# TheShadow29/VidSitu

Hardware: AMD Instinct MI355X
Metric: clips/s (10s@32x224x224) SlowFast+TxEnc fwd+bwd (higher is better)
Workload: dtype bf16

## Files before the change

### vidsitu_amd/csrc/conv_wgrad.hip

```cpp
#include <stdlib.h>

#include "common.h"

#include <mutex>
#include <type_traits>
#include "glue_bodies.h"

typedef __attribute__((ext_vector_type(4))) short s16x4;
typedef __attribute__((address_space(3))) s16x4 lds_s16x4;

struct WgradP {
  const uint16_t* dy;
  const uint16_t* x;
  float* out;
  int P;
  int Cout, Kp, Cin, x_ld, dy_ld;
  int To, Ho, Wo, Ti, Hi, Wi;
  int kT, kH, kW, sT, sH, sW, pT, pH, pW;
  int tilesM, tilesN, S, rows_per_split;
  unsigned x_bytes, dy_bytes;
  int xcd_order;
  int dbg;
};

#define WG_OOB 0x80000000u

#define WG_ROWTAB 1024

__device__ __forceinline__ int wg_swz_chunk(int row) {
  return ((row & 3) << 1) | (((row >> 3) & 1) << 3);
}

#ifndef WG_NARROW_DEPTH
#define WG_NARROW_DEPTH 3
#endif
constexpr int wg_depth(int bm) { return bm <= 32 ? WG_NARROW_DEPTH : 2; }

template <int BM, int BN, int WM, int WN, int MODE>
__global__ __launch_bounds__(256) void conv_wgrad_kernel(WgradP p) {
  extern __shared__ __attribute__((aligned(16))) char smem[];
  constexpr int D = wg_depth(BM), R = D - 1;
  static_assert(D >= 2 && R * 64 < WG_ROWTAB / 2, "loads never run past the table half being rebuilt");
  constexpr int TM = BM / WM, TN = BN / WN;
  constexpr int MR = TM / 16, NR = TN / 16;
  constexpr int CM = BM / 8, CN = BN / 8;
  constexpr int RPM = 256 / CM, RPN = 256 / CN;
  constexpr int IM = (64 + RPM - 1) / RPM, IN = (64 + RPN - 1) / RPN;
  constexpr int IMG = 64 * 256;
  constexpr int STAGE = 2 * IMG;
  static_assert(WM * WN == 4, "4 waves");

  const int tid = threadIdx.x;
  int bid = blockIdx.x;
  if (p.xcd_order) {
    const int nwg = gridDim.x, q = nwg >> 3, r = nwg & 7, xcd = blockIdx.x & 7;
    bid = (xcd < r ? xcd * (q + 1) : r * (q + 1) + (xcd - r) * q) + (blockIdx.x >> 3);
  }
  const int ntile = p.tilesM * p.tilesN;
  const int s = bid / ntile;
  bid -= s * ntile;
  const int tn = bid % p.tilesN, tm = bid / p.tilesN;
  const int m0 = tm * BM, n0 = tn * BN;
  const int pbeg = s * p.rows_per_split;
  const int pend = min(p.P, pbeg + p.rows_per_split);

  int4* rowtab = (int4*)(smem + 2 * STAGE);

  const int ccm = tid % CM, rm = tid / CM;
  const int ccn = tid % CN, rn = tid / CN;
  const bool mcol_ok = (m0 + ccm * 8) < p.Cout;
  const int ncol = n0 + ccn * 8;
  const bool ncol_ok = ncol < p.Kp;
  int dt = 0, dh = 0, dw = 0, c0 = 0;
  if (MODE == 1 && ncol_ok) {
    const int tap = ncol / p.Cin;
    c0 = ncol - tap * p.Cin;
    dw = tap % p.kW;
    const int t2 = tap / p.kW;
    dh = t2 % p.kH;
    dt = t2 / p.kH;
  }

  u32x4 ra[R][IM], rb[R][IN];
  const __amdgpu_buffer_rsrc_t xsrc =
      __builtin_amdgcn_make_buffer_rsrc((void*)p.x, 0, (int)p.x_bytes, 0x00020000);
  const __amdgpu_buffer_rsrc_t dysrc =
      __builtin_amdgcn_make_buffer_rsrc((void*)p.dy, 0, (int)p.dy_bytes, 0x00020000);
  const unsigned dycol = (unsigned)((m0 + ccm * 8) * 2);
  const unsigned xtap = (MODE == 1)
      ? (unsigned)(((((long long)dt * p.Hi + dh) * p.Wi + dw) * p.x_ld + c0) * 2)
      : (unsigned)(ncol * 2);

  auto gload_a = [&](int u, int pstep) __attribute__((always_inline)) {
#pragma unroll
    for (int i = 0; i < IM; ++i) {
      const int r = rm + RPM * i;
      const int pp = pstep + r;
      const unsigned ok = (unsigned)(r < 64) & (unsigned)mcol_ok & (unsigned)(pp < pend);
      const unsigned off = ok ? (unsigned)pp * (unsigned)(p.dy_ld * 2) + dycol : WG_OOB;
      ra[u][i] = __builtin_bit_cast(u32x4, __builtin_amdgcn_raw_buffer_load_b128(dysrc, off, 0, 0));
    }
  };
  auto gload_b = [&](int u, int pstep) __attribute__((always_inline)) {
#pragma unroll
    for (int i = 0; i < IN; ++i) {
      const int r = rn + RPN * i;
      const int pp = pstep + r;
      unsigned ok = (unsigned)(r < 64) & (unsigned)ncol_ok & (unsigned)(pp < pend);
      unsigned off;
      if (MODE == 0) {
        off = (unsigned)pp * (unsigned)(p.x_ld * 2) + xtap;
      } else {
        const int4 e = rowtab[(pp - pbeg) & (WG_ROWTAB - 1)];
        const int ti = e.y + dt, hi = e.z + dh, wi = e.w + dw;
        ok &= (unsigned)((unsigned)ti < (unsigned)p.Ti) & (unsigned)((unsigned)hi < (unsigned)p.Hi) &
              (unsigned)((unsigned)wi < (unsigned)p.Wi);
        off = (unsigned)e.x + xtap;
      }
      rb[u][i] = __builtin_bit_cast(u32x4, __builtin_amdgcn_raw_buffer_load_b128(xsrc, ok ? off : WG_OOB, 0, 0));
    }
  };

  auto sstore = [&](int u, int buf) __attribute__((always_inline)) {
    char* A = smem + buf * STAGE;
    char* B = A + IMG;
#pragma unroll
    for (int i = 0; i < IM; ++i) {
      const int r = rm + RPM * i;
      if (r < 64) *(u32x4*)(A + r * 256 + ((ccm ^ wg_swz_chunk(r)) << 4)) = ra[u][i];
    }
#pragma unroll
    for (int i = 0; i < IN; ++i) {
      const int r = rn + RPN * i;
      if (r < 64) *(u32x4*)(B + r * 256 + ((ccn ^ wg_swz_chunk(r)) << 4)) = rb[u][i];
    }
  };

  auto build_tab = [&](int rel0, int count) __attribute__((always_inline)) {
    for (int i = tid; i < count; i += 256) {
      const int pp = pbeg + rel0 + i;
      int4 e = make_int4(0, -(1 << 20), -(1 << 20), -(1 << 20));
      if (pp < pend) {
        int wo, t1, ho, t2, to, n;
        if (p.P < (1 << 24)) {
          fast_divmod(pp, p.Wo, 1.0f / (float)p.Wo, t1, wo);
          fast_divmod(t1, p.Ho, 1.0f / (float)p.Ho, t2, ho);
          fast_divmod(t2, p.To, 1.0f / (float)p.To, n, to);
        } else {
          wo = pp % p.Wo; t1 = pp / p.Wo;
          ho = t1 % p.Ho; t2 = t1 / p.Ho;
          to = t2 % p.To; n = t2 / p.To;
        }
        e.y = to * p.sT - p.pT;
        e.z = ho * p.sH - p.pH;
        e.w = wo * p.sW - p.pW;
        const long long pos0 = (((long long)n * p.Ti + e.y) * p.Hi + e.z) * p.Wi + e.w;
        e.x = (int)(unsigned)(pos0 * p.x_ld * 2);
      }
      rowtab[(rel0 + i) & (WG_ROWTAB - 1)] = e;
    }
  };

  const int wave = tid >> 6, lane = tid & 63;
  const int wm = wave / WN, wn = wave % WN;
  const int g = lane >> 4, li = lane & 15, q = li >> 2, pp4 = li & 3;

  f32x4 acc[MR][NR];
#pragma unroll
  for (int a = 0; a < MR; ++a)
#pragma unroll
    for (int b = 0; b < NR; ++b) acc[a][b] = (f32x4){0.f, 0.f, 0.f, 0.f};

  auto compute = [&](int buf) __attribute__((always_inline)) {
    const char* A = smem + buf * STAGE;
    const char* B = A + IMG;
#pragma unroll
    for (int ks = 0; ks < 2; ++ks) {
      const int row = ks * 32 + 8 * g + q;
      const int swz = ((row & 3) << 2) | (((row >> 3) & 1) << 4);
      bf16x8 af[MR], bfr[NR];
#pragma unroll
      for (int a = 0; a < MR; ++a) {
        const int unit = ((wm * TM + a * 16) >> 2) + pp4;
        const lds_s16x4* ptr = (const lds_s16x4*)(A + row * 256 + ((unit ^ swz) << 3));
        const s16x4 lo = __builtin_amdgcn_ds_read_tr16_b64_v4i16((lds_s16x4*)ptr);
        const s16x4 hi = __builtin_amdgcn_ds_read_tr16_b64_v4i16((lds_s16x4*)(ptr + 128));
        typedef __attribute__((ext_vector_type(8))) short s16x8;
        const s16x8 v = __builtin_shufflevector(lo, hi, 0, 1, 2, 3, 4, 5, 6, 7);
        af[a] = __builtin_bit_cast(bf16x8, v);
      }
#pragma unroll
      for (int b = 0; b < NR; ++b) {
        const int unit = ((wn * TN + b * 16) >> 2) + pp4;
        const lds_s16x4* ptr = (const lds_s16x4*)(B + row * 256 + ((unit ^ swz) << 3));
        const s16x4 lo = __builtin_amdgcn_ds_read_tr16_b64_v4i16((lds_s16x4*)ptr);
        const s16x4 hi = __builtin_amdgcn_ds_read_tr16_b64_v4i16((lds_s16x4*)(ptr + 128));
        typedef __attribute__((ext_vector_type(8))) short s16x8;
        const s16x8 v = __builtin_shufflevector(lo, hi, 0, 1, 2, 3, 4, 5, 6, 7);
        bfr[b] = __builtin_bit_cast(bf16x8, v);
      }
#pragma unroll
      for (int a = 0; a < MR; ++a)
#pragma unroll
        for (int b = 0; b < NR; ++b)
          acc[a][b] = __builtin_amdgcn_mfma_f32_16x16x32_bf16(af[a], bfr[b], acc[a][b], 0, 0, 0);
    }
  };

  if constexpr (D == 2) {
    for (int chunk0 = pbeg; chunk0 < pend; chunk0 += WG_ROWTAB) {
      const int cend = min(pend, chunk0 + WG_ROWTAB);
      if (MODE == 1) {
        __syncthreads();
        build_tab(chunk0 - pbeg, WG_ROWTAB);
        __syncthreads();
      }
      const int nsteps = (cend - chunk0 + 63) >> 6;
      gload_a(0, chunk0);
      gload_b(0, chunk0);
      __syncthreads();
      sstore(0, 0);
      __syncthreads();
      for (int st = 0; st < nsteps - 1; ++st) {
        const int cur = st & 1;
        gload_a(0, chunk0 + (st + 1) * 64);
        gload_b(0, chunk0 + (st + 1) * 64);
        __builtin_amdgcn_sched_barrier(0);
        compute(cur);
        __builtin_amdgcn_sched_barrier(0);
        sstore(0, cur ^ 1);
        __syncthreads();
      }
      compute((nsteps - 1) & 1);
      __syncthreads();
    }
  } else {
    constexpr int HALF = WG_ROWTAB / 2, SPH = HALF / 64;
    const int nsteps = (pend - pbeg + 63) >> 6;
#pragma unroll
    for (int u = 0; u < R; ++u) gload_a(u, pbeg + u * 64);
    if (MODE == 1) {
      build_tab(0, HALF);
      __syncthreads();
    }
#pragma unroll
    for (int u = 0; u < R; ++u) gload_b(u, pbeg + u * 64);
    sstore(0, 0);
    __syncthreads();
    auto iter = [&](int u, int st) __attribute__((always_inline)) {
      if (MODE == 1 && (st & (SPH - 1)) == 0 && pbeg + (st / SPH + 1) * HALF < pend) build_tab((st / SPH + 1) * HALF, HALF);
      gload_a(u, pbeg + (st + R) * 64);
      gload_b(u, pbeg + (st + R) * 64);
      __builtin_amdgcn_sched_barrier(0);
      compute(st & 1);
      __builtin_amdgcn_sched_barrier(0);
      sstore((u + 1) % R, (st + 1) & 1);
      __syncthreads();
    };
    int st = 0;
    for (; st + R < nsteps; st += R) {
#pragma unroll
      for (int u = 0; u < R; ++u) iter(u, st + u);
    }
#pragma unroll
    for (int u = 0; u < R - 1; ++u)
      if (st + u < nsteps - 1) iter(u, st + u);
    if (nsteps > 0) compute((nsteps - 1) & 1);
  }

  float* dst = p.out + (long long)s * p.Cout * p.Kp;
#pragma unroll
  for (int a = 0; a < MR; ++a)
#pragma unroll
    for (int b = 0; b < NR; ++b) {
      const int col = n0 + wn * TN + b * 16 + li;
#pragma unroll
      for (int r = 0; r < 4; ++r) {
        const int row = m0 + wm * TM + a * 16 + g * 4 + r;
        if (row < p.Cout && col < p.Kp) dst[(long long)row * p.Kp + col] = acc[a][b][r];
      }
    }
}

template <int BM, int BN, int WM, int WN, int MODE, int NS, int ROWS = 64>
__device__ __forceinline__ void conv_wgrad_ring_body(const WgradP& p, const int blk, const int nblk) {
  static_assert(ROWS == 64, "stage depth (the half-depth variant of round 4 was measured slower and removed)");
  extern __shared__ __attribute__((aligned(16))) char smem[];
  constexpr int TM = BM / WM, TN = BN / WN;
  constexpr int MR = TM / 16, NR = TN / 16;
  constexpr int CM = BM / 8, CN = BN / 8;
  constexpr int IMG = ROWS * 256;
  constexpr int STAGE = 2 * IMG;
  constexpr int D = NS - 1;
  constexpr int RG = ROWS / 16;
  constexpr int L = 2 * RG;
  constexpr int SPC = WG_ROWTAB / ROWS;
  static_assert(WM * WN == 4, "4 waves");
  static_assert((D - 1) * L <= 63, "vmcnt range");

  const int tid = threadIdx.x;
  int bid = blk;
  if (p.xcd_order) {
    const int nwg = nblk, q = nwg >> 3, r = nwg & 7, xcd = blk & 7;
    bid = (xcd < r ? xcd * (q + 1) : r * (q + 1) + (xcd - r) * q) + (blk >> 3);
  }
  const int ntile = p.tilesM * p.tilesN;
  const int s = bid / ntile;
  bid -= s * ntile;
  const int tn = bid % p.tilesN, tm = bid / p.tilesN;
  const int m0 = tm * BM, n0 = tn * BN;
  const int pbeg = s * p.rows_per_split;
  const int pend = min(p.P, pbeg + p.rows_per_split);
  const int nsteps = (pend - pbeg + ROWS - 1) / ROWS;
  int2* rowtab = (int2*)(smem + NS * STAGE);

  const int wv = __builtin_amdgcn_readfirstlane(tid >> 6), lane = tid & 63;
  const int rg = lane >> 4, cc = lane & 15;
  const int lc = cc ^ ((rg << 1) | ((wv >> 1) << 3));
  const bool mcol_ok = lc < CM && (m0 + lc * 8) < p.Cout;
  const int ncol = n0 + lc * 8;
  const bool ncol_ok = lc < CN && ncol < p.Kp;
  int tap = 0, c0 = 0, dt = 0, dh = 0, dw = 0;
  if (MODE == 1 && ncol_ok) {
    tap = ncol / p.Cin;
    c0 = ncol - tap * p.Cin;
    dw = tap % p.kW;
    const int t2 = tap / p.kW;
    dh = t2 % p.kH;
    dt = t2 / p.kH;
  }
  const unsigned dycol = (unsigned)((m0 + lc * 8) * 2);
  const unsigned xtap = (MODE == 1)
      ? (unsigned)(((((long long)dt * p.Hi + dh) * p.Wi + dw) * p.x_ld + c0) * 2)
      : (unsigned)(ncol * 2);
  const unsigned dy_pitch = (unsigned)(p.dy_ld * 2), x_pitch = (unsigned)(p.x_ld * 2);

  typedef __attribute__((address_space(3))) char* lds_ptr_t;
  const unsigned lds0 = (unsigned)(unsigned long)(lds_ptr_t)smem + (unsigned)wv * 1024u;
  auto rsrc_words = [](const void* base, unsigned bytes) __attribute__((always_inline)) {
    const unsigned long a = (unsigned long)base;
    return (i32x4){(int)(unsigned)a, (int)((unsigned)(a >> 32) & 0xffffu), (int)bytes, 0x00020000};
  };
  const i32x4 xdesc = rsrc_words(p.x, p.x_bytes), dydesc = rsrc_words(p.dy, p.dy_bytes);
  auto dma16 = [](const i32x4& desc, unsigned lds_addr, unsigned voff) __attribute__((always_inline)) {
    asm volatile("s_mov_b32 m0, %0\n\ts_nop 0\n\tbuffer_load_dwordx4 %1, %2, 0 offen lds"
                 :
                 : "s"(lds_addr), "v"(voff), "s"(desc)
                 : "memory");
  };

  const bool small_p = p.P < (1 << 24);
  const float rcpWo = 1.0f / (float)p.Wo, rcpHo = 1.0f / (float)p.Ho, rcpTo = 1.0f / (float)p.To;
  auto build_tab = [&](int chunk) __attribute__((always_inline)) {
    int2* tab = rowtab + (chunk & 1) * WG_ROWTAB;
    const int base = pbeg + chunk * WG_ROWTAB;
    for (int i = tid; i < WG_ROWTAB; i += 256) {
      const int pp = base + i;
      int2 e = make_int2(0, 0);
      if (pp < pend) {
        int wo, t1, ho, t2, to, n;
        if (small_p) {
          fast_divmod(pp, p.Wo, rcpWo, t1, wo);
          fast_divmod(t1, p.Ho, rcpHo, t2, ho);
          fast_divmod(t2, p.To, rcpTo, n, to);
        } else {
          wo = pp % p.Wo; t1 = pp / p.Wo;
          ho = t1 % p.Ho; t2 = t1 / p.Ho;
          to = t2 % p.To; n = t2 / p.To;
        }
        const int ti0 = to * p.sT - p.pT, hi0 = ho * p.sH - p.pH, wi0 = wo * p.sW - p.pW;
        const long long pos0 = (((long long)n * p.Ti + ti0) * p.Hi + hi0) * p.Wi + wi0;
        e.x = (int)(unsigned)(pos0 * p.x_ld * 2);
        unsigned mt = 0u, mh = 0u, mw = 0u;
        for (int a = 0; a < p.kT; ++a) mt |= ((unsigned)(ti0 + a) < (unsigned)p.Ti ? 1u : 0u) << a;
        for (int a = 0; a < p.kH; ++a) mh |= ((unsigned)(hi0 + a) < (unsigned)p.Hi ? 1u : 0u) << a;
        for (int a = 0; a < p.kW; ++a) mw |= ((unsigned)(wi0 + a) < (unsigned)p.Wi ? 1u : 0u) << a;
        unsigned mk = 0u;
        int tp = 0;
        for (int a = 0; a < p.kT; ++a)
          for (int b = 0; b < p.kH; ++b) {
            const unsigned th = (mt >> a) & (mh >> b) & 1u;
            mk |= (th ? mw : 0u) << tp;
            tp += p.kW;
          }
        e.y = (int)mk;
      }
      tab[i] = e;
    }
  };

  auto dma = [&](int st, int stage) __attribute__((always_inline)) {
    const unsigned A = lds0 + (unsigned)(stage * STAGE);
    const unsigned B = A + IMG;
    const int rel0 = st * ROWS + 4 * wv + rg;
    int2 ent[RG];
    if (MODE == 1) {
#pragma unroll
      for (int i = 0; i < RG; ++i) {
        const int rel = rel0 + 16 * i;
        ent[i] = rowtab[((rel >> 10) & 1) * WG_ROWTAB + (rel & (WG_ROWTAB - 1))];
      }
    }
#pragma unroll
    for (int i = 0; i < RG; ++i) {
      const int rel = rel0 + 16 * i;
      const int pp = pbeg + rel;
      const unsigned ok = (unsigned)mcol_ok & (unsigned)(pp < pend);
      dma16(dydesc, A + i * 4096, ok ? (unsigned)pp * dy_pitch + dycol : WG_OOB);
    }
#pragma unroll
    for (int i = 0; i < RG; ++i) {
      const int rel = rel0 + 16 * i;
      const int pp = pbeg + rel;
      unsigned ok = (unsigned)ncol_ok & (unsigned)(pp < pend);
      unsigned off;
      if (MODE == 0) {
        off = (unsigned)pp * x_pitch + xtap;
      } else {
        ok &= ((unsigned)ent[i].y >> tap) & 1u;
        off = (unsigned)ent[i].x + xtap;
      }
      dma16(xdesc, B + i * 4096, ok ? off : WG_OOB);
    }
  };

  const int wm = wv / WN, wn = wv % WN;
  const int g = lane >> 4, li = lane & 15, q = li >> 2, pp4 = li & 3;
  f32x4 acc[MR][NR];
#pragma unroll
  for (int a = 0; a < MR; ++a)
#pragma unroll
    for (int b = 0; b < NR; ++b) acc[a][b] = (f32x4){0.f, 0.f, 0.f, 0.f};

  auto compute = [&](int stage) __attribute__((always_inline)) {
    const char* A = smem + stage * STAGE;
    const char* B = A + IMG;
#pragma unroll
    for (int ks = 0; ks < ROWS / 32; ++ks) {
      const int row = ks * 32 + 8 * g + q;
      const int swz = ((row & 3) << 2) | (((row >> 3) & 1) << 4);
      bf16x8 af[MR], bfr[NR];
      typedef __attribute__((ext_vector_type(8))) short s16x8;
#pragma unroll
      for (int a = 0; a < MR; ++a) {
        const int unit = ((wm * TM + a * 16) >> 2) + pp4;
        const lds_s16x4* ptr = (const lds_s16x4*)(A + row * 256 + ((unit ^ swz) << 3));
        const s16x4 lo = __builtin_amdgcn_ds_read_tr16_b64_v4i16((lds_s16x4*)ptr);
        const s16x4 hi = __builtin_amdgcn_ds_read_tr16_b64_v4i16((lds_s16x4*)(ptr + 128));
        af[a] = __builtin_bit_cast(bf16x8, (s16x8)__builtin_shufflevector(lo, hi, 0, 1, 2, 3, 4, 5, 6, 7));
      }
#pragma unroll
      for (int b = 0; b < NR; ++b) {
        const int unit = ((wn * TN + b * 16) >> 2) + pp4;
        const lds_s16x4* ptr = (const lds_s16x4*)(B + row * 256 + ((unit ^ swz) << 3));
        const s16x4 lo = __builtin_amdgcn_ds_read_tr16_b64_v4i16((lds_s16x4*)ptr);
        const s16x4 hi = __builtin_amdgcn_ds_read_tr16_b64_v4i16((lds_s16x4*)(ptr + 128));
        bfr[b] = __builtin_bit_cast(bf16x8, (s16x8)__builtin_shufflevector(lo, hi, 0, 1, 2, 3, 4, 5, 6, 7));
      }
#pragma unroll
      for (int a = 0; a < MR; ++a)
#pragma unroll
        for (int b = 0; b < NR; ++b)
          acc[a][b] = __builtin_amdgcn_mfma_f32_16x16x32_bf16(af[a], bfr[b], acc[a][b], 0, 0, 0);
    }
  };

  if (MODE == 1) {
    build_tab(0);
    __syncthreads();
  }
#pragma unroll
  for (int d = 0; d < D; ++d) dma(d, d);
  int st_c = 0, st_l = D;
  for (int st = 0; st < nsteps; ++st) {
    if (!(p.dbg & 4)) asm volatile("s_waitcnt vmcnt(%0) lgkmcnt(0)" ::"i"((D - 1) * L) : "memory");
    if (!(p.dbg & 8)) __builtin_amdgcn_s_barrier();
    __builtin_amdgcn_sched_barrier(0);
    if (MODE == 1 && (st % SPC) == 0 && pbeg + (st / SPC + 1) * WG_ROWTAB < pend && !(p.dbg & 32))
      build_tab(st / SPC + 1);
    if (!(p.dbg & 2)) dma(st + D, st_l);
    __builtin_amdgcn_sched_barrier(0);
    if (!(p.dbg & 1)) compute(st_c);
    __builtin_amdgcn_sched_barrier(0);
    st_c = (st_c + 1 == NS) ? 0 : st_c + 1;
    st_l = (st_l + 1 == NS) ? 0 : st_l + 1;
  }
  asm volatile("s_waitcnt vmcnt(0)" ::: "memory");
  if ((p.dbg & 64) && acc[0][0][0] != 123.456f) return;

  float* dst = p.out + (long long)s * p.Cout * p.Kp;
#pragma unroll
  for (int a = 0; a < MR; ++a)
#pragma unroll
    for (int b = 0; b < NR; ++b) {
      const int col = n0 + wn * TN + b * 16 + li;
#pragma unroll
      for (int r = 0; r < 4; ++r) {
        const int row = m0 + wm * TM + a * 16 + g * 4 + r;
        if (row < p.Cout && col < p.Kp) dst[(long long)row * p.Kp + col] = acc[a][b][r];
// ... 193 lines not shown
  read_frags(0, FA0, FB0);
  close_phase();
  int slot = 0;
  auto phase = [&](auto par, int ph) __attribute__((always_inline)) {
    constexpr int PAR = decltype(par)::value;
    open_phase(ph + 1);
    if (MODE == 1 && (ph & 15) == 0 && pbeg + ((ph >> 4) + 1) * WGD_TAB < pend) build_tab((ph >> 4) + 1);
    if (!STAG || hf == 0) dma_unit(ph + 6, slot);
    const int nslot = slot + 1 == WGD_NU ? 0 : slot + 1;
    if (PAR == 0) {
      read_frags(nslot, FA1, FB1);
      mma(FA0, FB0);
    } else {
      read_frags(nslot, FA0, FB0);
      mma(FA1, FB1);
    }
    if (STAG && hf == 1) {
      __builtin_amdgcn_sched_barrier(0);
      dma_unit(ph + 6, slot);
    }
    close_phase();
    slot = nslot;
  };
  int ph = 0;
  for (; ph + 1 < nu; ph += 2) {
    phase(std::integral_constant<int, 0>{}, ph);
    phase(std::integral_constant<int, 1>{}, ph + 1);
  }
  if (ph < nu) phase(std::integral_constant<int, 0>{}, ph);
  asm volatile("s_waitcnt vmcnt(0)" ::: "memory");
  __syncthreads();

  float* E = (float*)smem;
#pragma unroll
  for (int a = 0; a < 4; ++a)
#pragma unroll
    for (int b = 0; b < 4; ++b) {
      const int col = wn * 64 + b * 16 + li;
#pragma unroll
      for (int r = 0; r < 4; ++r) E[(wm * 64 + a * 16 + g * 4 + r) * WGD_EP + col] = acc[a][b][r];
    }
  __syncthreads();
  float* dst = p.out + (long long)s * p.Cout * p.Kp;
  for (int idx = tid; idx < 128 * 64; idx += 512) {
    const int row = idx >> 6, c4 = idx & 63;
    if (m0 + row < p.Cout && n0 + c4 * 4 < p.Kp)
      *(float4*)(dst + (long long)(m0 + row) * p.Kp + n0 + c4 * 4) = *(const float4*)(E + row * WGD_EP + c4 * 4);
  }
}

template <int MODE, bool STAG>
__global__ __launch_bounds__(512) void conv_wgrad_deep_kernel(WgradP p) {
  conv_wgrad_deep_body<MODE, STAG>(p, blockIdx.x, gridDim.x);
}

#define WGG_MAX 20
#define WGG_JOBS 16
struct WgGroupP {
  int n;
  int first[WGG_MAX + 1];
  int count[WGG_MAX];
  int mode[WGG_MAX];
  int jobs;
  unsigned short jobend[8];
  unsigned jobtab[8][WGG_JOBS];
  WgradP p[WGG_MAX];
};
static_assert(sizeof(WgGroupP) <= 4096, "kernel arguments");

__global__ __launch_bounds__(512) void conv_wgrad_deep_group_kernel(WgGroupP g) {
  const int b = blockIdx.x;
  if (g.jobs) {
    const int xcd = b & 7, slot = b >> 3;
    unsigned e = ~0u;
    int jend = 0;
#pragma unroll
    for (int x = 0; x < 8; ++x) {
      const bool mine = x == xcd;
      jend = mine ? (int)g.jobend[x] : jend;
#pragma unroll
      for (int i = 0; i < WGG_JOBS; ++i) {
        const unsigned t = g.jobtab[x][i];
        if (mine && (int)(t >> 23) <= slot) e = t;
      }
    }
    if (slot >= jend) return;
    const int j = __builtin_amdgcn_readfirstlane((int)((e >> 18) & 31));
    const int sp = (int)((e >> 12) & 63), tile0 = (int)(e & 4095);
    const int tile = tile0 + slot - (int)(e >> 23);
    const int blk = __builtin_amdgcn_readfirstlane(sp * (g.p[j].tilesM * g.p[j].tilesN) + tile);
#ifdef VS_WGG_DEBUG
    if (j >= g.n || sp >= g.p[j].S || tile >= g.p[j].tilesM * g.p[j].tilesN) {
      if (threadIdx.x == 0) printf("bad job: b %d xcd %d slot %d e %x j %d sp %d tile %d (n %d S %d nt %d)\n", b, xcd, slot, e, j, sp, tile, g.n, g.p[j].S, g.p[j].tilesM * g.p[j].tilesN);
      return;
    }
#endif
    if (g.mode[j] == 0) conv_wgrad_deep_body<0, true>(g.p[j], blk, g.count[j]);
    else conv_wgrad_deep_body<1, true>(g.p[j], blk, g.count[j]);
    return;
  }
  int j = 0;
#pragma unroll
  for (int i = 1; i < WGG_MAX; ++i)
    if (i < g.n && b >= g.first[i]) j = i;
  j = __builtin_amdgcn_readfirstlane(j);
  const int lo = g.first[j], cnt = g.count[j];
  if (b - lo >= cnt) return;
  if (g.mode[j] == 0) conv_wgrad_deep_body<0, true>(g.p[j], b - lo, cnt);
  else conv_wgrad_deep_body<1, true>(g.p[j], b - lo, cnt);
}

struct WgReduceGroupP {
  int n;
  long long first[WGG_MAX + 1];
  const float* slabs[WGG_MAX];
  float* dw[WGG_MAX];
  long long len[WGG_MAX];
  int S[WGG_MAX];
};

__global__ __launch_bounds__(256) void wgrad_reduce_group_kernel(WgReduceGroupP g) {
  __shared__ float4 part[16][17];
  const long long b = blockIdx.x;
  int e = 0;
#pragma unroll
  for (int i = 1; i < WGG_MAX; ++i)
    if (i < g.n && b >= g.first[i]) e = i;
  wgrad_reduce_body(g.slabs[e], g.dw[e], g.len[e], g.S[e], part, b - g.first[e], threadIdx.x);
}

__global__ __launch_bounds__(256) void wgrad_reduce_kernel(const float* slabs, float* dw,
                                                          long long n, int S) {
  __shared__ float4 part[16][17];
  wgrad_reduce_body(slabs, dw, n, S, part, blockIdx.x, threadIdx.x);
}

namespace {
struct PendingState {
  int mode = 0;
  bool have = false;
  VsPendingReduce r{};
};
thread_local PendingState g_pending;

static void pending_launch(const VsPendingReduce& r) {
  const long long grid = wgrad_reduce_vblocks(r.n, r.S);
  hipLaunchKernelGGL(wgrad_reduce_kernel, dim3((unsigned)grid), dim3(256), 0, r.st, r.slabs, r.dw, r.n, r.S);
}
}

static void pending_flush() {
  if (g_pending.have) {
    g_pending.have = false;
    pending_launch(g_pending.r);
  }
}

static bool pending_stash(const float* slabs, float* dw, long long n, int S, hipStream_t st) {
  if (g_pending.mode != 1) return false;
  pending_flush();
  g_pending.r = VsPendingReduce{slabs, dw, n, S, st};
  g_pending.have = true;
  return true;
}

bool vs_pending_reduce_take(hipStream_t st, VsPendingReduce* out) {
  if (!g_pending.have || g_pending.r.st != st) return false;
  *out = g_pending.r;
  g_pending.have = false;
  return true;
}

extern "C" int vs_wgrad_reduce_defer(int mode) {
  VS_CHECK_ARG(mode >= 0 && mode <= 2, "mode 0 (off), 1 (defer), 2 (suspend)");
  if (mode == 0) pending_flush();
  g_pending.mode = mode;
  VS_CHECK_LAUNCH();
  return VS_OK;
}

extern "C" int vs_wgrad_reduce_flush(void) {
  pending_flush();
  VS_CHECK_LAUNCH();
  return VS_OK;
}

__global__ __launch_bounds__(256) void wgrad_reduce_batched_kernel(const long long* __restrict__ table, int nent) {
  __shared__ float4 part[16][17];
  const long long b = blockIdx.x;
  int lo = 0, hi = nent - 1;
  while (lo < hi) {
    const int mid = (lo + hi + 1) >> 1;
    if (table[mid * 5 + 4] <= b) lo = mid; else hi = mid - 1;
  }
  const float* slabs = (const float*)table[lo * 5 + 0];
  float* dw = (float*)table[lo * 5 + 1];
  const long long n = table[lo * 5 + 2];
  const int S = (int)table[lo * 5 + 3];
  const long long blk = b - table[lo * 5 + 4];
  const long long n4 = n >> 2;
  const int col = threadIdx.x & 15, sl = threadIdx.x >> 4;
  const long long i = blk * 16 + col;
  float4 acc = make_float4(0.f, 0.f, 0.f, 0.f);
  if (i < n4) {
    const int per = (S + 15) / 16;
    const int s0 = sl * per, s1 = min(S, s0 + per);
    int s = s0;
    for (; s + 8 <= s1; s += 8) {
      float4 v[8];
#pragma unroll
      for (int u = 0; u < 8; ++u) v[u] = *(const float4*)(slabs + (long long)(s + u) * n + i * 4);
#pragma unroll
      for (int u = 0; u < 8; ++u) {
        acc.x += v[u].x;
        acc.y += v[u].y;
        acc.z += v[u].z;
        acc.w += v[u].w;
      }
    }
    for (; s < s1; ++s) {
      const float4 v = *(const float4*)(slabs + (long long)s * n + i * 4);
      acc.x += v.x;
      acc.y += v.y;
      acc.z += v.z;
      acc.w += v.w;
    }
  }
  part[sl][col] = acc;
  __syncthreads();
  if (sl == 0 && i < n4) {
    float4 t = part[0][col];
    for (int k = 1; k < 16; ++k) {
      const float4 v = part[k][col];
      t.x += v.x;
      t.y += v.y;
      t.z += v.z;
      t.w += v.w;
    }
    *(float4*)(dw + i * 4) = t;
  }
}

extern "C" int vs_wgrad_reduce_batched(const int64_t* table, int n_entries, int64_t total_blocks, void* stream) {
  VS_CHECK_ARG(table && n_entries > 0 && total_blocks > 0, "bad args");
  hipLaunchKernelGGL(wgrad_reduce_batched_kernel, dim3((unsigned)total_blocks), dim3(256), 0, (hipStream_t)stream,
                     (const long long*)table, n_entries);
  VS_CHECK_LAUNCH();
  return VS_OK;
}

extern "C" int64_t vs_wgrad_reduce_blocks(int64_t n) { return (n / 4 + 15) / 16; }

extern "C" int vs_wgrad_reduce(const float* slabs, float* dw, int64_t n, int splits, void* stream) {
  VS_CHECK_ARG(slabs && dw && n > 0 && splits > 1, "bad args");
  hipLaunchKernelGGL(wgrad_reduce_kernel, dim3((unsigned)wgrad_reduce_vblocks(n, splits)), dim3(256), 0, (hipStream_t)stream,
                     slabs, dw, (long long)n, splits);
  VS_CHECK_LAUNCH();
  return VS_OK;
}

struct WgCfg {
  int bm, bn, S, rows_per_split, tilesM, tilesN;
  int deep;
};


static bool wg_deep_plan(const vs_conv_desc* d, WgCfg* c) {
  static const int mode = [] { const char* e = getenv("VS_WGRAD_DEEP"); return e ? atoi(e) : 1; }();
  const bool force = mode == 2 || (d->flags & VS_WGRAD_FORCEDEEP);
  if (mode == 0 || (d->flags & VS_WGRAD_NODEEP)) return false;
  if (((d->flags >> 8) & 0xf) || ((d->flags >> 16) & 7) || ((d->flags >> 24) & 0xff)) return false;
  const int taps = d->kT * d->kH * d->kW;
  const int Kp = taps * d->Cin;
  const long long P = (long long)d->N * d->To * d->Ho * d->Wo;
  if (taps > 31 || Kp % 8 != 0 || d->Cout % 8 != 0) return false;
  const int tilesM = (d->Cout + 127) / 128, tilesN = (Kp + 255) / 256;
  const long long tiles = (long long)tilesM * tilesN;
  const double row_eff = (double)d->Cout / (128.0 * tilesM), col_eff = (double)Kp / (256.0 * tilesN);
  long long S = 256 / tiles;
  const long long maxS = P / 512;
  if (S > maxS) S = maxS;
  const long long slab_cap = (64ll << 20) / ((long long)d->Cout * Kp * 4);
  if (S > slab_cap) S = slab_cap;
  if (S < 1) S = 1;
  long long rps = (P + S - 1) / S;
  rps = (rps + 31) / 32 * 32;
  S = (P + rps - 1) / rps;
  if (!force && (row_eff < 0.9 || col_eff < 0.75 || tiles * S < 128 || tiles > 256 || rps < 512)) return false;
  static const long long min_p = [] { const char* e = getenv("VS_WGRAD_DEEP_MINP"); return e ? atoll(e) : 3000ll; }();
  if (!force && P < min_p) return false;
  if (tiles * S > 65535) return false;
  c->bm = 128;
  c->bn = 256;
  c->tilesM = tilesM;
  c->tilesN = tilesN;
  c->S = (int)S;
  c->rows_per_split = (int)rps;
  c->deep = 1;
  return true;
}

static const int kWgTiles[8][2] = {{128, 128}, {128, 64}, {64, 128}, {64, 64}, {32, 128}, {32, 64}, {16, 128}, {16, 64}};

static WgCfg wg_pick(const vs_conv_desc* d) {
  WgCfg c;
  c.deep = 0;
  if (wg_deep_plan(d, &c)) return c;
  const int Kp = d->kT * d->kH * d->kW * d->Cin;
  const long long P = (long long)d->N * d->To * d->Ho * d->Wo;
  c.bm = d->Cout >= 128 ? 128 : (d->Cout >= 64 ? 64 : (d->Cout >= 32 ? 32 : 16));
  c.bn = Kp >= 128 ? 128 : 64;
  if (d->Cout <= 16) c.bn = Kp > 64 ? 128 : 64;
  else if (d->Cout <= 32) c.bn = 64;
  const int forced = (d->flags >> 8) & 0xf;
  if (forced >= 1 && forced <= 8) {
    c.bm = kWgTiles[forced - 1][0];
    c.bn = kWgTiles[forced - 1][1];
  }
  c.tilesM = (d->Cout + c.bm - 1) / c.bm;
  c.tilesN = (Kp + c.bn - 1) / c.bn;
  const long long tiles = (long long)c.tilesM * c.tilesN;
  static const long long slots = [] {
    const char* e = getenv("VS_WGRAD_SLOTS");
    return e ? atoll(e) : 384ll;
  }();
  static const long long small_slots = [] {
    const char* e = getenv("VS_WGRAD_SLOTS_SMALL");
    return e ? atoll(e) : 512ll;
  }();
  long long target = (d->Cout <= 32) ? small_slots : slots;
  const int forced_slots = (d->flags >> 24) & 0xff;
  if (forced_slots) target = 8ll * forced_slots;
  long long S = target / tiles;
  static const long long s1_tiles = [] {
    const char* e = getenv("VS_WGRAD_S1_TILES");
    return e ? atoll(e) : 128ll;
  }();
  if (s1_tiles > 0 && tiles >= s1_tiles && !forced_slots) S = 1;
  const long long maxS = (P + 511) / 512;
  if (S > maxS) S = maxS;
  const long long slab_cap = (64ll << 20) / ((long long)d->Cout * Kp * 4);
  if (S > slab_cap) S = slab_cap;
  if (S > 1024) S = 1024;
  if (S < 1) S = 1;
  long long rps = (P + S - 1) / S;
  rps = (rps + 63) / 64 * 64;
  S = (P + rps - 1) / rps;
  c.S = (int)S;
  c.rows_per_split = (int)rps;
  return c;
}

extern "C" size_t vs_conv_wgrad_workspace_bytes(const vs_conv_desc* d) {
  const WgCfg c = wg_pick(d);
  if (c.S <= 1) return 0;
  return (size_t)c.S * d->Cout * d->kT * d->kH * d->kW * d->Cin * sizeof(float);
}

static bool pair_take_wgrad(const WgradP& p, int grid, size_t smem, int mode, hipStream_t st);
static bool pair_defer_reduce(const float* slabs, float* dw, long long n, int splits);
#ifndef VS_CONV_PAIR_TU
static bool pair_take_wgrad(const WgradP&, int, size_t, int, hipStream_t) { return false; }
static bool pair_defer_reduce(const float*, float*, long long, int) { return false; }
#endif

template <int BM, int BN, int WM, int WN>
static int wg_launch(const WgradP& p, int mode, int ring, hipStream_t st) {
  const int grid = p.tilesM * p.tilesN * p.S;
  static bool attr_done = false;
  if (!attr_done) {
    (void)hipFuncSetAttribute((const void*)conv_wgrad_kernel<BM, BN, WM, WN, 0>,
                              hipFuncAttributeMaxDynamicSharedMemorySize, 160 * 1024);
    (void)hipFuncSetAttribute((const void*)conv_wgrad_kernel<BM, BN, WM, WN, 1>,
                              hipFuncAttributeMaxDynamicSharedMemorySize, 160 * 1024);
    (void)hipFuncSetAttribute((const void*)conv_wgrad_ring_kernel<BM, BN, WM, WN, 0, 2>,
                              hipFuncAttributeMaxDynamicSharedMemorySize, 160 * 1024);
    (void)hipFuncSetAttribute((const void*)conv_wgrad_ring_kernel<BM, BN, WM, WN, 1, 2>,
                              hipFuncAttributeMaxDynamicSharedMemorySize, 160 * 1024);
    (void)hipFuncSetAttribute((const void*)conv_wgrad_ring_kernel<BM, BN, WM, WN, 0, 3>,
                              hipFuncAttributeMaxDynamicSharedMemorySize, 160 * 1024);
    (void)hipFuncSetAttribute((const void*)conv_wgrad_ring_kernel<BM, BN, WM, WN, 1, 3>,
                              hipFuncAttributeMaxDynamicSharedMemorySize, 160 * 1024);
    attr_done = true;
  }
  if (ring >= 2) {
    const size_t tab = mode ? 2 * WG_ROWTAB * sizeof(int2) : 0;
    const size_t smem = (size_t)ring * 2 * 64 * 256 + tab;
    if constexpr (BM == 128 && BN == 128) {
      if (ring == 2 && pair_take_wgrad(p, grid, smem, mode, st)) return VS_OK;
    }
    if (ring == 2 && mode == 0)
      hipLaunchKernelGGL((conv_wgrad_ring_kernel<BM, BN, WM, WN, 0, 2>), dim3(grid), dim3(256), smem, st, p);
    else if (ring == 2)
      hipLaunchKernelGGL((conv_wgrad_ring_kernel<BM, BN, WM, WN, 1, 2>), dim3(grid), dim3(256), smem, st, p);
    else if (mode == 0)
      hipLaunchKernelGGL((conv_wgrad_ring_kernel<BM, BN, WM, WN, 0, 3>), dim3(grid), dim3(256), smem, st, p);
    else
      hipLaunchKernelGGL((conv_wgrad_ring_kernel<BM, BN, WM, WN, 1, 3>), dim3(grid), dim3(256), smem, st, p);
    VS_CHECK_LAUNCH();
    return VS_OK;
  }
  const size_t smem = 2 * 2 * 64 * 256 + (mode ? WG_ROWTAB * sizeof(int4) : 0);
  if (mode == 0)
    hipLaunchKernelGGL((conv_wgrad_kernel<BM, BN, WM, WN, 0>), dim3(grid), dim3(256), smem, st, p);
  else
    hipLaunchKernelGGL((conv_wgrad_kernel<BM, BN, WM, WN, 1>), dim3(grid), dim3(256), smem, st, p);
  VS_CHECK_LAUNCH();
  return VS_OK;
}

static int wg_fill_params(WgradP& p, const void* dy, const void* x, float* out, const vs_conv_desc* d, const WgCfg& c) {
  p.dy = (const uint16_t*)dy;
  p.x = (const uint16_t*)x;
  p.out = out;
  p.P = d->N * d->To * d->Ho * d->Wo;
  p.Cout = d->Cout;
  p.Cin = d->Cin;
  p.Kp = d->kT * d->kH * d->kW * d->Cin;
  p.x_ld = d->x_ld;
  p.dy_ld = d->y_ld;
  p.To = d->To; p.Ho = d->Ho; p.Wo = d->Wo;
  p.Ti = d->Ti; p.Hi = d->Hi; p.Wi = d->Wi;
  p.kT = d->kT; p.kH = d->kH; p.kW = d->kW;
  p.sT = d->sT; p.sH = d->sH; p.sW = d->sW;
  p.pT = d->pT; p.pH = d->pH; p.pW = d->pW;
  {
    const long long xb = (long long)d->N * d->Ti * d->Hi * d->Wi * d->x_ld * 2;
    const long long db = (long long)p.P * d->y_ld * 2;
    VS_CHECK_ARG(xb < (1ll << 31) && db < (1ll << 31), "tensor larger than 2 GiB");
    p.x_bytes = (unsigned)xb;
    p.dy_bytes = (unsigned)db;
  }
  p.tilesM = c.tilesM;
  p.tilesN = c.tilesN;
  p.S = c.S;
  p.rows_per_split = c.rows_per_split;
  p.xcd_order = 0;
  p.dbg = 0;
  return VS_OK;
}

static bool wgg_item_ok(const vs_conv_desc* d) {
  const int taps = d->kT * d->kH * d->kW;
  const long long Kp = (long long)taps * d->Cin;
  if (taps > 31 || Kp % 8 != 0 || d->Cout % 8 != 0 || d->x_ld % 8 != 0 || d->y_ld % 8 != 0) return false;
  if (((d->flags >> 8) & 0xf) || ((d->flags >> 16) & 7) || ((d->flags >> 24) & 0xff)) return false;
  const long long P = (long long)d->N * d->To * d->Ho * d->Wo;
  const long long xb = (long long)d->N * d->Ti * d->Hi * d->Wi * d->x_ld * 2;
  const long long db = P * d->y_ld * 2;
  return P >= 512 && xb < (1ll << 31) && db < (1ll << 31);
}

#define WGG_C0 14
static bool wgg_plan(const vs_wgrad_item* it, int n, WgCfg* cfg, size_t* slab_off, size_t* slab_total, int* order) {
  if (n < 1 || n > WGG_MAX) return false;
  static const int slots = [] { const char* e = getenv("VS_WGG_SLOTS"); const int v = e ? atoi(e) : 256; return v < 1 ? 1 : (v > 1024 ? 1024 : v); }();
  long long units[WGG_MAX], P[WGG_MAX], maxS[WGG_MAX], dwn[WGG_MAX];
  int tiles[WGG_MAX];
  long long W = 0, umax = 0;
  for (int j = 0; j < n; ++j) {
    const vs_conv_desc* d = &it[j].d;
    if (!wgg_item_ok(d)) return false;
    const int Kp = d->kT * d->kH * d->kW * d->Cin;
    cfg[j].bm = 128;
    cfg[j].bn = 256;
    cfg[j].deep = 1;
    cfg[j].tilesM = (d->Cout + 127) / 128;
    cfg[j].tilesN = (Kp + 255) / 256;
    tiles[j] = cfg[j].tilesM * cfg[j].tilesN;
    P[j] = (long long)d->N * d->To * d->Ho * d->Wo;
    units[j] = (P[j] + 31) / 32;
    dwn[j] = (long long)d->Cout * Kp;
    maxS[j] = P[j] / 512;
    const long long slab_cap = (64ll << 20) / (dwn[j] * 4);
    if (maxS[j] > slab_cap) maxS[j] = slab_cap;
    if (maxS[j] < 1) maxS[j] = 1;
    W += (long long)tiles[j] * units[j];
    if (units[j] > umax) umax = units[j];
  }
  auto splits = [&](long long u, long long* S, long long* rps) {
    for (int j = 0; j < n; ++j) {
      long long s = (units[j] + u / 2) / u;
      if (s > maxS[j]) s = maxS[j];
      if (s < 1) s = 1;
      long long r = (P[j] + s - 1) / s;
      r = (r + 31) / 32 * 32;
      S[j] = (P[j] + r - 1) / r;
      rps[j] = r;
    }
  };
  auto cost = [&](const long long* S, const long long* rps) {
    int ord[WGG_MAX];
    for (int j = 0; j < n; ++j) ord[j] = j;
    for (int a = 0; a < n; ++a)
      for (int b = a + 1; b < n; ++b)
        if (rps[ord[b]] > rps[ord[a]]) { const int t = ord[a]; ord[a] = ord[b]; ord[b] = t; }
    long long slot[1024];
    for (int i = 0; i < slots; ++i) slot[i] = 0;
    long long span = 0;
    int nxt = 0;
    for (int a = 0; a < n; ++a) {
      const int j = ord[a];
      const long long len = WGG_C0 + (rps[j] + 31) / 32;
      const long long nb = (long long)tiles[j] * S[j];
      for (long long b = 0; b < nb; ++b) {
        int best = nxt;
        if ((b % slots) == 0) {
          for (int i = 0; i < slots; ++i)
            if (slot[i] < slot[best]) best = i;
        }
        slot[best] += len;
        if (slot[best] > span) span = slot[best];
        nxt = (best + 1) % slots;
      }
    }
    double slab = 0.0;
    for (int j = 0; j < n; ++j)
      if (S[j] > 1) slab += 2.0 * (double)S[j] * (double)dwn[j] * 4.0;
    return (double)span + slab / 3.0e12 / 0.64e-6;
  };
  long long bestS[WGG_MAX], bestR[WGG_MAX], S[WGG_MAX], R[WGG_MAX];
  double best = -1.0;
  long long u = W / (3ll * slots);
  if (u < 16) u = 16;
  if (u > umax) u = umax;
  for (; u <= umax + 1; u += (u + 15) / 16) {
    splits(u, S, R);
    const double c = cost(S, R);
    if (best < 0.0 || c < best) {
      best = c;
      for (int j = 0; j < n; ++j) { bestS[j] = S[j]; bestR[j] = R[j]; }
    }
  }
  if (best < 0.0) return false;
  size_t off = 0;
  long long blocks = 0;
  for (int j = 0; j < n; ++j) {
    cfg[j].S = (int)bestS[j];
    cfg[j].rows_per_split = (int)bestR[j];
    slab_off[j] = off;
    if (bestS[j] > 1) off += (size_t)bestS[j] * dwn[j] * sizeof(float);
    blocks += (long long)tiles[j] * bestS[j];
    order[j] = j;
  }
  for (int a = 0; a < n; ++a)
    for (int b = a + 1; b < n; ++b)
      if (bestR[order[b]] > bestR[order[a]]) { const int t = order[a]; order[a] = order[b]; order[b] = t; }
  *slab_total = off;
  return blocks <= 65535;
}

extern "C" int vs_conv_wgrad_group_ok(const vs_wgrad_item* items, int n) {
  if (items == nullptr) return 0;
  WgCfg cfg[WGG_MAX];
  size_t off[WGG_MAX], tot;
  int order[WGG_MAX];
  return wgg_plan(items, n, cfg, off, &tot, order) ? 1 : 0;
}

extern "C" size_t vs_conv_wgrad_group_workspace_bytes(const vs_wgrad_item* items, int n) {
  if (items == nullptr) return 0;
  WgCfg cfg[WGG_MAX];
  size_t off[WGG_MAX], tot = 0;
  int order[WGG_MAX];
  if (!wgg_plan(items, n, cfg, off, &tot, order)) return 0;
  return tot;
}

extern "C" int vs_conv_wgrad_group(const vs_wgrad_item* items, int n, void* workspace, size_t ws_bytes, void* stream) {
  VS_CHECK_ARG(items != nullptr && n >= 1 && n <= WGG_MAX, "1 .. 20 items");
  WgCfg cfg[WGG_MAX];
  size_t off[WGG_MAX], tot = 0;
  int order[WGG_MAX];
  if (!wgg_plan(items, n, cfg, off, &tot, order)) {
    vs_set_error("vs_conv_wgrad_group: an item is outside the deep-pipeline kernel's envelope (ask vs_conv_wgrad_group_ok)");
    return VS_ERR_UNSUPPORTED;
  }
  if (tot > 0 && (workspace == nullptr || ws_bytes < tot)) {
    vs_set_error("vs_conv_wgrad_group: workspace too small (%zu < %zu)", ws_bytes, tot);
    return VS_ERR_WORKSPACE;
  }
  if (g_pending.have) pending_flush();
  WgGroupP g;
  WgReduceGroupP r;
  g.n = n;
  r.n = 0;
  r.first[0] = 0;
  int first = 0;
  for (int a = 0; a < n; ++a) {
    const int j = order[a];
    const vs_wgrad_item& t = items[j];
    VS_CHECK_ARG(t.dy && t.x && t.dw, "null tensor");
    const vs_conv_desc* d = &t.d;
    float* out = cfg[j].S > 1 ? (float*)((char*)workspace + off[j]) : t.dw;
    const int rc = wg_fill_params(g.p[a], t.dy, t.x, out, d, cfg[j]);
    if (rc) return rc;
    const bool dense = (d->kT * d->kH * d->kW == 1) && d->sT == 1 && d->sH == 1 && d->sW == 1 && d->pT == 0 &&
                       d->pH == 0 && d->pW == 0;
    g.mode[a] = dense ? 0 : 1;
    g.first[a] = first;
    g.count[a] = cfg[j].tilesM * cfg[j].tilesN * cfg[j].S;
    first += g.count[a];
    if (cfg[j].S > 1) {
      const int e = r.n++;
      r.slabs[e] = out;
      r.dw[e] = t.dw;
      r.len[e] = (long long)d->Cout * g.p[a].Kp;
      r.S[e] = cfg[j].S;
      r.first[e + 1] = r.first[e] + wgrad_reduce_vblocks(r.len[e], r.S[e]);
    }
  }
  g.first[n] = first;
  for (int j = n; j < WGG_MAX; ++j) g.first[j + 1] = first;
  g.jobs = 0;
  int grid = first;
  {
    static const int jobs_on = [] { const char* e = getenv("VS_WGG_JOBS"); return e ? atoi(e) : 0; }();
    bool fits = jobs_on != 0 && n <= 32;
    int cnt[8] = {0, 0, 0, 0, 0, 0, 0, 0};
    for (int x = 0; x < 8; ++x) {
      g.jobend[x] = 0;
      for (int i = 0; i < WGG_JOBS; ++i) g.jobtab[x][i] = ~0u;
    }
    long long pos = 0;
    for (int a = 0; a < n && fits; ++a) {
      const int nt = g.p[a].tilesM * g.p[a].tilesN;
      if (nt > 4095 || g.p[a].S > 63) { fits = false; break; }
      for (int sp = 0; sp < g.p[a].S && fits; ++sp) {
        int t0 = 0;
        while (t0 < nt) {
          const long long chunk = pos >> 5;
          const int room = 32 - (int)(pos & 31), c = nt - t0 < room ? nt - t0 : room;
          const int x = (int)(chunk & 7), slot0 = (int)(chunk >> 3) * 32 + (int)(pos & 31);
          if (cnt[x] == WGG_JOBS || slot0 + c > 510) { fits = false; break; }
          g.jobtab[x][cnt[x]++] = ((unsigned)slot0 << 23) | ((unsigned)a << 18) | ((unsigned)sp << 12) | (unsigned)t0;
          t0 += c;
          pos += c;
        }
      }
    }
    if (fits) {
      const long long chunks = (pos + 31) >> 5;
      int mx = 0;
      for (int x = 0; x < 8; ++x) {
        long long sl = 0;
        for (long long c = x; c < chunks; c += 8) sl = (c >> 3) * 32 + ((c == chunks - 1 && (pos & 31)) ? (pos & 31) : 32);
        g.jobend[x] = (unsigned short)sl;
        if ((int)sl > mx) mx = (int)sl;
      }
#ifdef VS_WGG_DEBUG
      for (int x = 0; x < 8; ++x) {
        fprintf(stderr, "xcd %d (%d slots):", x, (int)g.jobend[x]);
        for (int i = 0; i < cnt[x]; ++i) fprintf(stderr, " [slot %u p %u s %u t %u]", g.jobtab[x][i] >> 23, (g.jobtab[x][i] >> 18) & 31, (g.jobtab[x][i] >> 12) & 63, g.jobtab[x][i] & 4095);
        fprintf(stderr, "\n");
      }
      for (int a = 0; a < n; ++a) fprintf(stderr, "problem %d: tiles %d x %d S %d rps %d count %d\n", a, g.p[a].tilesM, g.p[a].tilesN, g.p[a].S, g.p[a].rows_per_split, g.count[a]);
#endif
      g.jobs = 1;
      grid = 8 * mx;
    }
  }
  static std::once_flag gattr;
  std::call_once(gattr, [] {
    (void)hipFuncSetAttribute((const void*)conv_wgrad_deep_group_kernel, hipFuncAttributeMaxDynamicSharedMemorySize, 160 * 1024);
  });
  const size_t smem = (size_t)WGD_NU * WGD_UNIT + 2 * WGD_TAB * sizeof(int2);
  hipLaunchKernelGGL(conv_wgrad_deep_group_kernel, dim3(grid), dim3(512), smem, (hipStream_t)stream, g);
  VS_CHECK_LAUNCH();
  if (r.n > 0) {
    hipLaunchKernelGGL(wgrad_reduce_group_kernel, dim3((unsigned)r.first[r.n]), dim3(256), 0, (hipStream_t)stream, r);
    VS_CHECK_LAUNCH();
  }
  return VS_OK;
}

static int wgrad_impl(const void* dy, const void* x, float* dw, const vs_conv_desc* d, void* workspace,
                      size_t ws_bytes, void* stream, bool reduce_now, int* splits_out) {
  VS_CHECK_ARG(d && dy && x && dw, "null argument");
  VS_CHECK_ARG(d->Cin % 8 == 0 && d->Cout % 8 == 0, "Cin and Cout must be multiples of 8");
  VS_CHECK_ARG(d->x_ld % 8 == 0 && d->y_ld % 8 == 0, "row pitches must be multiples of 8");
  VS_CHECK_ARG((long long)d->N * d->Ti * d->Hi * d->Wi < (1ll << 31), "too many positions");
  const WgCfg c = wg_pick(d);
  const size_t need = vs_conv_wgrad_workspace_bytes(d);
  if (need > 0 && (workspace == nullptr || ws_bytes < need)) {
    vs_set_error("vs_conv_wgrad: workspace too small (%zu < %zu)", ws_bytes, need);
    return VS_ERR_WORKSPACE;
  }
  if (g_pending.have && ((const void*)g_pending.r.slabs == workspace || g_pending.r.dw == dw)) pending_flush();
  WgradP p;
  {
    const int rc = wg_fill_params(p, dy, x, c.S > 1 ? (float*)workspace : dw, d, c);
    if (rc) return rc;
  }
  {
    static const int xo = [] { const char* e = getenv("VS_WGRAD_XCD"); return e ? atoi(e) : 1; }();
    p.xcd_order = xo && (c.tilesM * c.tilesN <= 32 || xo == 2 || (c.S % 8 == 0 && c.tilesM * c.tilesN <= 64));
    static const int dbg = [] { const char* e = getenv("VS_WGRAD_DBG"); return e ? atoi(e) : 0; }();
    p.dbg = dbg;
  }
  p.rows_per_split = c.rows_per_split;
  const bool dense = (d->kT * d->kH * d->kW == 1) && d->sT == 1 && d->sH == 1 && d->sW == 1 &&
                     d->pT == 0 && d->pH == 0 && d->pW == 0;
  const int mode = dense ? 0 : 1;
  hipStream_t st = (hipStream_t)stream;
  const int fring = (d->flags >> 16) & 7;
// ... 55 lines not shown
```

Before: 743.5.

## Size wgrad LDS staging images to tile width with per-pitch swizzle

The non-ring wgrad kernel used to stage every A and B tile in a fixed 256-byte-pitch LDS image, whatever BM and BN were. Images are now sized to the actual tile width (pitch = 2*cols). Each pitch gets its own XOR swizzle for the stores and for the transposed ds_read_tr16 loads, and the launch requests only the LDS it needs. The goal is a smaller LDS footprint for narrow tiles, so more workgroups can be resident per CU. The risk is new bank conflicts from the narrow-pitch swizzles, and possible mismatches between the store and read addressing.

Result: no change. 745.7, median of 6 (+0.3%).

```diff
diff --git a/vidsitu_amd/csrc/conv_wgrad.hip b/vidsitu_amd/csrc/conv_wgrad.hip
--- a/vidsitu_amd/csrc/conv_wgrad.hip
+++ b/vidsitu_amd/csrc/conv_wgrad.hip
@@ -36,6 +36,27 @@
 #endif
 constexpr int wg_depth(int bm) { return bm <= 32 ? WG_NARROW_DEPTH : 2; }
 
+constexpr int wg_img_bytes(int cols) { return 64 * cols * 2; }
+constexpr int wg_stage_bytes(int bm, int bn) { return wg_img_bytes(bm) + wg_img_bytes(bn); }
+constexpr int wg_lds_bytes(int bm, int bn, int mode) {
+  return 2 * wg_stage_bytes(bm, bn) + (mode ? WG_ROWTAB * (int)sizeof(int4) : 0);
+}
+
+template <int PITCH>
+__device__ __forceinline__ int wg_img_off(int row, int unit) {
+  static_assert(PITCH == 32 || PITCH == 64 || PITCH == 128 || PITCH == 256, "16 .. 128 channels per row");
+  const int b3 = (row >> 3) & 1;
+  if constexpr (PITCH == 32) return (row ^ (b3 << 2)) * PITCH + (unit << 3);
+  const int x = PITCH == 256 ? ((row & 3) | (b3 << 2)) : PITCH == 128 ? (((row >> 1) & 1) | (b3 << 1)) : b3;
+  return row * PITCH + ((unit ^ (x << 2)) << 3);
+}
+
+template <int PITCH>
+__device__ __forceinline__ int wg_img_hi(int row, int unit) {
+  if constexpr (PITCH == 32) return wg_img_off<PITCH>(row + 4, unit);
+  return wg_img_off<PITCH>(row, unit) + 4 * PITCH;
+}
+
 template <int BM, int BN, int WM, int WN, int MODE>
 __global__ __launch_bounds__(256) void conv_wgrad_kernel(WgradP p) {
   extern __shared__ __attribute__((aligned(16))) char smem[];
@@ -46,8 +67,9 @@
   constexpr int CM = BM / 8, CN = BN / 8;
   constexpr int RPM = 256 / CM, RPN = 256 / CN;
   constexpr int IM = (64 + RPM - 1) / RPM, IN = (64 + RPN - 1) / RPN;
-  constexpr int IMG = 64 * 256;
-  constexpr int STAGE = 2 * IMG;
+  constexpr int PA = BM * 2, PB = BN * 2;
+  constexpr int IMGA = wg_img_bytes(BM);
+  constexpr int STAGE = wg_stage_bytes(BM, BN);
   static_assert(WM * WN == 4, "4 waves");
 
   const int tid = threadIdx.x;
@@ -123,16 +145,16 @@
 
   auto sstore = [&](int u, int buf) __attribute__((always_inline)) {
     char* A = smem + buf * STAGE;
-    char* B = A + IMG;
+    char* B = A + IMGA;
 #pragma unroll
     for (int i = 0; i < IM; ++i) {
       const int r = rm + RPM * i;
-      if (r < 64) *(u32x4*)(A + r * 256 + ((ccm ^ wg_swz_chunk(r)) << 4)) = ra[u][i];
+      if (r < 64) *(u32x4*)(A + wg_img_off<PA>(r, ccm * 2)) = ra[u][i];
     }
 #pragma unroll
     for (int i = 0; i < IN; ++i) {
       const int r = rn + RPN * i;
-      if (r < 64) *(u32x4*)(B + r * 256 + ((ccn ^ wg_swz_chunk(r)) << 4)) = rb[u][i];
+      if (r < 64) *(u32x4*)(B + wg_img_off<PB>(r, ccn * 2)) = rb[u][i];
     }
   };
 
@@ -173,18 +195,17 @@
 
   auto compute = [&](int buf) __attribute__((always_inline)) {
     const char* A = smem + buf * STAGE;
-    const char* B = A + IMG;
+    const char* B = A + IMGA;
+    const int row = 8 * g + q;
 #pragma unroll
     for (int ks = 0; ks < 2; ++ks) {
-      const int row = ks * 32 + 8 * g + q;
-      const int swz = ((row & 3) << 2) | (((row >> 3) & 1) << 4);
       bf16x8 af[MR], bfr[NR];
 #pragma unroll
       for (int a = 0; a < MR; ++a) {
         const int unit = ((wm * TM + a * 16) >> 2) + pp4;
-        const lds_s16x4* ptr = (const lds_s16x4*)(A + row * 256 + ((unit ^ swz) << 3));
-        const s16x4 lo = __builtin_amdgcn_ds_read_tr16_b64_v4i16((lds_s16x4*)ptr);
-        const s16x4 hi = __builtin_amdgcn_ds_read_tr16_b64_v4i16((lds_s16x4*)(ptr + 128));
+        const char* img = A + ks * 32 * PA;
+        const s16x4 lo = __builtin_amdgcn_ds_read_tr16_b64_v4i16((lds_s16x4*)(img + wg_img_off<PA>(row, unit)));
+        const s16x4 hi = __builtin_amdgcn_ds_read_tr16_b64_v4i16((lds_s16x4*)(img + wg_img_hi<PA>(row, unit)));
         typedef __attribute__((ext_vector_type(8))) short s16x8;
         const s16x8 v = __builtin_shufflevector(lo, hi, 0, 1, 2, 3, 4, 5, 6, 7);
         af[a] = __builtin_bit_cast(bf16x8, v);
@@ -192,9 +213,9 @@
 #pragma unroll
       for (int b = 0; b < NR; ++b) {
         const int unit = ((wn * TN + b * 16) >> 2) + pp4;
-        const lds_s16x4* ptr = (const lds_s16x4*)(B + row * 256 + ((unit ^ swz) << 3));
-        const s16x4 lo = __builtin_amdgcn_ds_read_tr16_b64_v4i16((lds_s16x4*)ptr);
-        const s16x4 hi = __builtin_amdgcn_ds_read_tr16_b64_v4i16((lds_s16x4*)(ptr + 128));
+        const char* img = B + ks * 32 * PB;
+        const s16x4 lo = __builtin_amdgcn_ds_read_tr16_b64_v4i16((lds_s16x4*)(img + wg_img_off<PB>(row, unit)));
+        const s16x4 hi = __builtin_amdgcn_ds_read_tr16_b64_v4i16((lds_s16x4*)(img + wg_img_hi<PB>(row, unit)));
         typedef __attribute__((ext_vector_type(8))) short s16x8;
         const s16x8 v = __builtin_shufflevector(lo, hi, 0, 1, 2, 3, 4, 5, 6, 7);
         bfr[b] = __builtin_bit_cast(bf16x8, v);
@@ -994,6 +1015,7 @@
 
 static const int kWgTiles[8][2] = {{128, 128}, {128, 64}, {64, 128}, {64, 64}, {32, 128}, {32, 64}, {16, 128}, {16, 64}};
 
+
 static WgCfg wg_pick(const vs_conv_desc* d) {
   WgCfg c;
   c.deep = 0;
@@ -1092,7 +1114,7 @@
     VS_CHECK_LAUNCH();
     return VS_OK;
   }
-  const size_t smem = 2 * 2 * 64 * 256 + (mode ? WG_ROWTAB * sizeof(int4) : 0);
+  const size_t smem = (size_t)wg_lds_bytes(BM, BN, mode);
   if (mode == 0)
     hipLaunchKernelGGL((conv_wgrad_kernel<BM, BN, WM, WN, 0>), dim3(grid), dim3(256), smem, st, p);
   else
```
